# gnlpfjh/Scalable-E3-GNN

Measured on AMD Instinct MI355X. Metric: particles/sec (octree build + SEGNN fwd), 1M pts l_max=2, 1/2/4/8 MI355X, higher is better.
Workload: dtype f32; 1 GPU; 1000000 particles/GPU uniform in unit box, radius graph k~24 (E=23519616), SEGNN l_max=2 4 layers H=32 f32 storage; particles_per_gpu=1000000, edges_per_gpu=23519616, hidden=32, layers=4, lmax=2, parallelism=single GPU

## Files before the change

### include/e3gnn.h

```cpp
#ifndef E3GNN_H
#define E3GNN_H

#include <stdint.h>

#ifdef __cplusplus
extern "C" {
#endif

#define E3GNN_ABI_VERSION 3

enum {
  E3_OK = 0,
  E3_ERR_INVALID_ARG = 1,
  E3_ERR_BAD_IRREPS = 2,
  E3_ERR_MISSING_WEIGHT = 3,
  E3_ERR_UNSUPPORTED = 4,
  E3_ERR_HIP = 5,
  E3_ERR_NO_DEVICE = 6
};

enum { E3_F32 = 0, E3_F64 = 1, E3_BF16 = 2 };

enum { E3_CLS_0E = 0, E3_CLS_0O = 1, E3_CLS_1E = 2, E3_CLS_1O = 3 };

// ... 122 lines not shown
int e3_pow2_scale(const e3_tp_segment* segs, const int64_t* nrows, int nseg, int target_log2, float* out4,
                  void* stream);
int e3_add_pow2_scale(const float* h, const float* u, float* out, int64_t n, int target_log2, float* out4,
                      void* stream);
int e3_tp_forward_fused(const e3_tp_plan* plan, const e3_tp_segment* segs, int nseg,
                        const void* in2, int64_t ld_in2, const void* packed, void* out, int64_t ld_out,
                        int64_t B, int dtype, int gate, const float* in_scale, void* stream);
int e3_tp_forward_fused_epilogue(const e3_tp_plan* plan, const e3_tp_segment* segs, int nseg, const void* in2,
                                 int64_t ld_in2, const void* packed, void* out, int64_t ld_out, int64_t B, int dtype,
                                 int gate, const float* in_scale, const void* residual, int64_t ld_residual,
                                 float* out_scale4, int target_log2, void* stream);
int e3_tp_forward_update_pair(const e3_tp_plan* plan1, const e3_tp_plan* plan2, const e3_tp_segment* segs, int nseg,
                              const void* in2, int64_t ld_in2, const void* packed1, const void* packed2,
                              const float* in_scale, const void* residual, int64_t ld_residual, void* out,
                              int64_t ld_out, int64_t B, int dtype, float* out_scale4, int target_log2, void* stream);
int e3_tp_backward(const e3_tp_plan* plan, const void* in1, int64_t ld_in1, const void* in2, int64_t ld_in2,
                   const void* packed, const void* grad_out, int64_t ld_gout, void* grad_in1, int64_t ld_gin1,
                   void* grad_in2, int64_t ld_gin2, void* const grad_weights[6], int64_t B, int dtype, void* stream);
int e3_tp_backward_weights(const e3_tp_plan* plan, const void* in1, int64_t ld_in1, const void* in2, int64_t ld_in2,
                           const void* packed, const void* grad_out, int64_t ld_gout, void* const grad_weights[6],
                           int64_t B, int dtype, void* stream);
int e3_tp_backward_operands(const e3_tp_plan* plan, const void* in1, int64_t ld_in1, const void* in2, int64_t ld_in2,
                            const void* packed, const void* grad_out, int64_t ld_gout, void* const features[6],
                            void* const gout[6], int64_t B, int dtype, void* stream);
int e3_tp_backward_contract(const e3_tp_plan* plan, const void* in1, int64_t ld_in1, const void* in2, int64_t ld_in2,
                            void* const t[6], void* grad_in1, int64_t ld_gin1, void* grad_in2, int64_t ld_gin2,
                            int64_t B, int dtype, void* stream);
int e3_tp_fused_supported(const e3_tp_plan* plan, int gate);
const char* e3_tp_last_fused_kernel(void);
int e3_tp_forward_fused_scatter(const e3_tp_plan* plan, const e3_tp_segment* segs, int nseg,
// ... 59 lines not shown
```

### scalable-e3-gnn_amd/_lib.py

```python
from __future__ import annotations

import ctypes
import os
from ctypes import POINTER, c_char_p, c_int, c_int32, c_int64, c_void_p

_HERE = os.path.dirname(os.path.abspath(__file__))
LIB_PATH = os.path.join(_HERE, "lib", "libe3gnn_hip.so")

E3_OK = 0
E3_F32, E3_F64, E3_BF16 = 0, 1, 2
CLS_NAMES = ("l0e", "l0o", "l1e", "l1o")

_lib = None

VoidP4 = c_void_p * 4
Float3 = ctypes.c_float * 3
Int3 = c_int32 * 3


class HaloEntry(ctypes.Structure):
    _fields_ = [("lo", ctypes.c_float * 3), ("hi", ctypes.c_float * 3), ("shift", ctypes.c_float * 3)]


SIGNATURES = {
# ... 81 lines not shown
    "e3_pow2_scale": (c_int, [c_void_p, POINTER(c_int64), c_int, c_int, c_void_p, c_void_p]),
    "e3_add_pow2_scale": (c_int, [c_void_p, c_void_p, c_void_p, c_int64, c_int, c_void_p, c_void_p]),
    "e3_tp_backward": (c_int, [c_void_p, c_void_p, c_int64, c_void_p, c_int64, c_void_p, c_void_p, c_int64, c_void_p,
                               c_int64, c_void_p, c_int64, c_void_p * 6, c_int64, c_int, c_void_p]),
    "e3_tp_backward_weights": (c_int, [c_void_p, c_void_p, c_int64, c_void_p, c_int64, c_void_p, c_void_p, c_int64, c_void_p,
                                       c_int64, c_int, c_void_p]),
    "e3_tp_backward_operands": (c_int, [c_void_p, c_void_p, c_int64, c_void_p, c_int64, c_void_p, c_void_p, c_int64, c_void_p,
                                        c_void_p, c_int64, c_int, c_void_p]),
    "e3_tp_backward_contract": (c_int, [c_void_p, c_void_p, c_int64, c_void_p, c_int64, c_void_p, c_void_p, c_int64, c_void_p,
                                        c_int64, c_int64, c_int, c_void_p]),
    "e3_tp_forward_fused_epilogue": (c_int, [c_void_p, c_void_p, c_int, c_void_p, c_int64, c_void_p, c_void_p, c_int64,
                                             c_int64, c_int, c_int, c_void_p, c_void_p, c_int64, c_void_p, c_int, c_void_p]),
    "e3_tp_forward_update_pair": (c_int, [c_void_p, c_void_p, c_void_p, c_int, c_void_p, c_int64, c_void_p, c_void_p,
                                          c_void_p, c_void_p, c_int64, c_void_p, c_int64, c_int64, c_int, c_void_p, c_int,
                                          c_void_p]),
    "e3_tp_fused_supported": (c_int, [c_void_p, c_int]),
    "e3_tp_last_fused_kernel": (ctypes.c_char_p, []),
    "e3_tp_forward_fused_scatter": (c_int, [c_void_p, c_void_p, c_int, c_void_p, c_int64, c_void_p, c_void_p, c_void_p,
                                            c_int64, c_int64, c_int, c_int, c_void_p, c_void_p]),
    "e3_segment_sum_bf16": (c_int, [c_void_p, c_int64, c_void_p, c_int64, c_int, c_void_p, c_int64, c_void_p]),
    "e3_edge_geometry_l2": (c_int, [c_void_p, c_void_p, c_void_p, c_int64, c_void_p, c_void_p, c_void_p, c_void_p]),
    "e3_gate_blocks": (c_int, [c_void_p, c_int64, c_void_p, c_int64, c_int64, c_int, c_int, POINTER(c_int32),
                               POINTER(c_int32), c_void_p]),
    "e3_l1tp_backward": (c_int, [c_void_p, c_void_p, c_int64, c_void_p, c_int64, VoidP4, VoidP4, c_void_p, c_int64,
                                 c_void_p, c_int64, c_void_p, VoidP4, c_void_p, c_int64, c_int, c_void_p]),
    "e3_edge_geometry_strained": (c_int, [c_void_p, c_void_p, c_void_p, c_int64, c_int, POINTER(ctypes.c_float), c_void_p,
                                          c_void_p, c_int, c_void_p, c_void_p, c_void_p, c_void_p]),
    "e3_edge_geometry_backward_strained_workspace_bytes": (c_int64, [c_int64]),
    "e3_edge_geometry_backward_strained": (c_int, [c_void_p, c_void_p, c_void_p, c_int64, c_int, POINTER(ctypes.c_float),
                                                   c_void_p, c_void_p, c_int, c_void_p, c_void_p, c_void_p, c_void_p,
# ... 100 lines not shown
```

### scalable-e3-gnn_amd/csrc/e3_tp.hip

```cpp
#include "e3_common.h"
#include "cg_tables.h"
#include "e3_tp_internal.h"

#include <algorithm>
#include <cstdlib>
#include <map>
#include <mutex>
#include <utility>

namespace e3 {

static int tp_ensure_dyn_lds(const void* fn, size_t bytes) {
  if (bytes <= 64 * 1024) return E3_OK;
  static std::mutex mu;
  static std::map<std::pair<const void*, int>, size_t> have;
  int dev = 0;
  if (hipGetDevice(&dev) != hipSuccess) return E3_ERR_HIP;
  std::lock_guard<std::mutex> lock(mu);
  size_t& cur = have[std::make_pair(fn, dev)];
  if (bytes > cur) {
    if (hipFuncSetAttribute(fn, hipFuncAttributeMaxDynamicSharedMemorySize, (int)bytes) != hipSuccess) return E3_ERR_HIP;
    cur = bytes;
  }
  return E3_OK;
// ... 1112 lines not shown
  if ((dtype != E3_F32 && dtype != E3_BF16) || !plan->fast.usable || ld2 == 0) return E3_ERR_UNSUPPORTED;
  hipStream_t s = (hipStream_t)stream;
  if (out_scale4) E3_HIP_CHECK(hipMemsetAsync(out_scale4, 0, 16, s));
  if (B > 0) {
    if (!in2 || !packed || !out || ld2 < plan->dev.Dy) return E3_ERR_INVALID_ARG;
    int st = tp_ensure_device(plan);
    if (st != E3_OK) return st;
    st = fast_forward(&plan->fast, segs, nseg, plan->dev.D1, in2, ld2, (const char*)packed + fast_section_offset(plan), out,
                      ldo, B, gate, dtype, plan->dev.ocol, in_scale, s, nullptr, residual, ld_residual,
                      out_scale4 ? reinterpret_cast<uint32_t*>(out_scale4) + 2 : nullptr);
    if (st != E3_OK) return st;
  }
  return out_scale4 ? scale_finalize(out_scale4, target_log2, s) : E3_OK;
}

int e3_tp_forward_update_pair(const e3_tp_plan* plan1, const e3_tp_plan* plan2, const e3_tp_segment* segs, int nseg,
                              const void* in2, int64_t ld2, const void* packed1, const void* packed2,
                              const float* in_scale, const void* residual, int64_t ld_residual, void* out, int64_t ldo,
                              int64_t B, int dtype, float* out_scale4, int target_log2, void* stream) {
  if (!plan1 || !plan2 || !segs || B < 0 || (residual && ld_residual <= 0)) return E3_ERR_INVALID_ARG;
  if (out_scale4 && (target_log2 < -20 || target_log2 > 14)) return E3_ERR_INVALID_ARG;
  if ((dtype != E3_F32 && dtype != E3_BF16) || ld2 == 0 || !e3::r16_pair_supported(&plan1->fast, &plan2->fast))
    return E3_ERR_UNSUPPORTED;
  if (!in2 || !packed1 || !packed2 || !out || ld2 < plan1->dev.Dy || ldo < plan2->dev.Dout) return E3_ERR_INVALID_ARG;
  hipStream_t s = (hipStream_t)stream;
  int st = tp_ensure_device(plan1);
  if (st == E3_OK) st = tp_ensure_device(plan2);
  if (st != E3_OK) return st;
  if (out_scale4) E3_HIP_CHECK(hipMemsetAsync(out_scale4, 0, 16, s));
  if (B > 0) {
    st = fast_forward_pair(&plan1->fast, &plan2->fast, segs, nseg, plan1->dev.D1, in2, ld2,
                           (const char*)packed1 + fast_section_offset(plan1), (const char*)packed2 + fast_section_offset(plan2),
                           out, ldo, B, dtype, plan1->dev.ocol, plan2->dev.ocol, in_scale, residual, ld_residual,
                           out_scale4 ? reinterpret_cast<uint32_t*>(out_scale4) + 2 : nullptr, s);
    if (st != E3_OK) return st;
  }
  return out_scale4 ? scale_finalize(out_scale4, target_log2, s) : E3_OK;
}

int e3_tp_forward_fused_scatter(const e3_tp_plan* plan, const e3_tp_segment* segs, int nseg, const void* in2,
                                int64_t ld2, const void* packed, const int32_t* row_node, void* out_nodes,
                                int64_t ldo, int64_t B, int dtype, int gate, const float* in_scale, void* stream) {
  if (!plan || !segs || !row_node || B < 0) return E3_ERR_INVALID_ARG;
  if ((dtype != E3_F32 && dtype != E3_BF16) || !gate || !plan->fast.usable || ld2 == 0) return E3_ERR_UNSUPPORTED;
  if (B == 0) return E3_OK;
  if (!in2 || !packed || !out_nodes || ld2 < plan->dev.Dy) return E3_ERR_INVALID_ARG;
  int st = tp_ensure_device(plan);
  if (st != E3_OK) return st;
  return fast_forward(&plan->fast, segs, nseg, plan->dev.D1, in2, ld2, (const char*)packed + fast_section_offset(plan),
                      out_nodes, ldo, B, gate, dtype, plan->dev.ocol, in_scale, (hipStream_t)stream, row_node);
}

// ... 102 lines not shown
```

### scalable-e3-gnn_amd/csrc/e3_tp_internal.h

```cpp
#pragma once
#include "e3_common.h"

#include <array>
#include <vector>

namespace e3 {

struct TpPath { int c1, l1, l2, wrow; };

struct FChunk {
  int col, count, l1;
  int wblk[3][3];
  int S[2], rows_per[2], inv[2];
};
struct FDev {
  int Dout, Dy, nchunks, ntab, lsh;
  int M[3], NT[3], Mpad[3], ooff[3];
  int bfoff[3];
  int bftotal;
};
struct FPack { int l3, orig_row, count, wblk; };

struct TpFast {
  FDev dev;
// ... 19 lines not shown
                 const float* in_scale, hipStream_t s, const int32_t* scatter = nullptr, const void* residual = nullptr,
                 int64_t ldr = 0, uint32_t* amax = nullptr);
int scale_finalize(float* out4, int target_log2, hipStream_t s);

void fast_note_kernel(const char* name);
const char* fast_last_kernel();

bool fast_gate_shape_ok(const TpFast* F);
bool r16_supported(const TpFast* F);
int fast_forward_r16(const TpFast* F, const void* seg_args, const void* in2, int64_t ld2, const void* packed, void* out,
                     int64_t ldo, int64_t B, int gate, int io16, const int32_t* ocol_tab, const float* in_scale,
                     hipStream_t s);
bool r16_pair_supported(const TpFast* F1, const TpFast* F2);
int fast_forward_pair_r16(const TpFast* F1, const TpFast* F2, const void* seg_args, const void* in2, int64_t ld2,
                          const void* packed1, const void* packed2, void* out, int64_t ldo, int64_t B, int io16,
                          const int32_t* ocol1, const int32_t* ocol2, const float* in_scale, hipStream_t s);
int fast_forward_pair(const TpFast* F1, const TpFast* F2, const e3_tp_segment* segs, int nseg, int D1, const void* in2,
                      int64_t ld2, const void* packed1, const void* packed2, void* out, int64_t ldo, int64_t B, int dtype,
                      const int32_t* ocol1, const int32_t* ocol2, const float* in_scale, const void* residual,
                      int64_t ldr, uint32_t* amax, hipStream_t s);

}
```

### scalable-e3-gnn_amd/csrc/e3_tp_mfma.hip

```cpp
#include "e3_common.h"
#include "e3_tp_internal.h"

#include <algorithm>
#include <cstdlib>
#include <vector>

namespace e3 {

#include "e3_tp_mfma_core.h"

template <typename T>
__global__ void fast_absmax_kernel(const T* w0, int64_t n0, const T* w1, int64_t n1, const T* w2, int64_t n2,
                                   uint32_t* hdr) {
  const T* w[3] = {w0, w1, w2};
  const int64_t n[3] = {n0, n1, n2};
  float m = 0.f;
  for (int c = 0; c < 3; ++c)
    for (int64_t i = blockIdx.x * (int64_t)blockDim.x + threadIdx.x; i < n[c]; i += (int64_t)gridDim.x * blockDim.x)
      m = fmax_finite(m, to_acc(w[c][i]));
  for (int o = 32; o > 0; o >>= 1) m = fmaxf(m, __shfl_xor(m, o));
  if ((threadIdx.x & 63) == 0 && m > 0.f) atomicMax(hdr, __builtin_bit_cast(uint32_t, m));
}

template <typename T>
// ... 197 lines not shown
                 uint32_t* amax) {
  if (!F->usable) return E3_ERR_UNSUPPORTED;
  const bool io16 = dtype == E3_BF16;
  SegArgs sa;
  const int st = fast_seg_args(F, segs, nseg, D1, ldo, scatter, residual, ldr, amax, sa);
  if (st != E3_OK) return st;
  if (gate && !fast_gate_shape_ok(F)) return E3_ERR_UNSUPPORTED;
  const int r = fast_forward_r16(F, &sa, in2, ld2, packed, out, ldo, B, gate, io16 ? 1 : 0, ocol_tab, in_scale, s);
  if (r == 1) return E3_OK;
  return r < 0 ? -r : E3_ERR_UNSUPPORTED;
}

int fast_forward_pair(const TpFast* F1, const TpFast* F2, const e3_tp_segment* segs, int nseg, int D1, const void* in2,
                      int64_t ld2, const void* packed1, const void* packed2, void* out, int64_t ldo, int64_t B, int dtype,
                      const int32_t* ocol1, const int32_t* ocol2, const float* in_scale, const void* residual,
                      int64_t ldr, uint32_t* amax, hipStream_t s) {
  if (!F1->usable || !F2->usable || !r16_pair_supported(F1, F2)) return E3_ERR_UNSUPPORTED;
  SegArgs sa;
  const int st = fast_seg_args(F1, segs, nseg, D1, ldo, nullptr, residual, ldr, amax, sa);
  if (st != E3_OK) return st;
  const int r = fast_forward_pair_r16(F1, F2, &sa, in2, ld2, packed1, packed2, out, ldo, B, dtype == E3_BF16 ? 1 : 0,
                                      ocol1, ocol2, in_scale, s);
  if (r == 1) return E3_OK;
  return r < 0 ? -r : E3_ERR_UNSUPPORTED;
}

}
```

### scalable-e3-gnn_amd/csrc/e3_tp_mfma_r16.hip

```cpp
#include "e3_common.h"
#include "cg_tables.h"
#include "e3_tp_internal.h"

#include <algorithm>
#include <cstdlib>
#include <mutex>
#include <type_traits>
#include <utility>
#include <vector>

namespace e3 {

#include "e3_tp_mfma_core.h"

template <int NT16, bool IO16, int STRIDE>
__device__ __forceinline__ void mma_group(const uint4 (&ah)[NT16], const uint4 (&al)[IO16 ? 1 : NT16], const uint4 bh,
                                          const uint4 bl, f32x4* acc) {
  if constexpr (IO16) {
#pragma unroll
    for (int t = 0; t < NT16; ++t)
      acc[t * STRIDE] = mfma16(__builtin_bit_cast(bf16x8, ah[t]), __builtin_bit_cast(bf16x8, bh), acc[t * STRIDE]);
  } else {
#pragma unroll
    for (int t = 0; t < NT16; ++t)
// ... 35 lines not shown
#pragma unroll
      for (int e = 0; e < 8; ++e) {
        const uint32_t w = w4[e >> 1];
        (&x[0][0])[8 * u + e] = __builtin_bit_cast(float, (e & 1) ? (w & 0xffff0000u) : (w << 16));
      }
    }
  } else {
    const float4* xv = reinterpret_cast<const float4*>(xr + 8 * g * D1);
#pragma unroll
    for (int u = 0; u < 2 * D1; ++u) {
      const float4 v = xv[u];
      (&x[0][0])[4 * u + 0] = v.x * xs; (&x[0][0])[4 * u + 1] = v.y * xs;
      (&x[0][0])[4 * u + 2] = v.z * xs; (&x[0][0])[4 * u + 3] = v.w * xs;
    }
  }
}

template <int L1, int L2, int L3, int NT16, bool IO16>
__device__ __forceinline__ void run16(const float (&x)[8][2 * L1 + 1], const bool live,
                                      const uint4* __restrict__ whi, const uint4* __restrict__ wlo,
                                      const float (&y)[9], f32x4 (&acc)[NT16][2 * L3 + 1]) {
  constexpr int D1 = 2 * L1 + 1, D2 = 2 * L2 + 1, D3 = 2 * L3 + 1;
  using C = CG<L1, L2, L3>;
  __builtin_amdgcn_sched_barrier(0);
  uint4 ah[NT16], al[IO16 ? 1 : NT16];
#pragma unroll
  for (int t = 0; t < NT16; ++t) {
    ah[t] = whi[16 * t];
    if constexpr (!IO16) al[t] = wlo[16 * t];
  }
// ... 431 lines not shown
  }
  if constexpr (!SCAT) {
    if (segs.amax) {
#pragma unroll
      for (int o = 32; o > 0; o >>= 1) amax = fmaxf(amax, __shfl_xor(amax, o, 64));
      if (lane == 0 && amax > 0.f) atomicMax(segs.amax, __builtin_bit_cast(uint32_t, amax));
    }
  }
}

struct PairArgs {
  const float* packed;
  const FDev* dp;
  const FChunk* chunks;
  const int32_t* ocol_tab;
};
constexpr int kPairTarget = 10;

template <int LSH, int NT0, int NT1, int NT2, int MODE, int... L1S>
__global__ __launch_bounds__(256, 2) void tp_update_pair_r16_kernel(SegArgs segs, const float* __restrict__ in2, int64_t ld2,
                                                                    const float* __restrict__ packed,
                                                                    void* __restrict__ outv, int64_t ldo, int64_t B,
                                                                    const FDev* __restrict__ dp,
                                                                    const FChunk* __restrict__ chunks,
                                                                    const int32_t* __restrict__ ocol_tab,
                                                                    const float* __restrict__ in_scale, PairArgs pr) {
  constexpr bool IO16 = MODE == 2;
  constexpr int NL = (NT1 > 0 ? 1 : 0) + (NT2 > 0 ? 1 : 0);
  static_assert(NT1 == 1 && NT2 <= 1 && NT0 == 1 + NL, "hidden 32: scalars and one gate block per degree, one tile each");
  constexpr int CHUNK = r16_chunk(r16_max({L1S...}), NL);
// ... 94 lines not shown
    stage(0);

    f32x4 a0[2 * NT0][1], a1[2][3], a2[NT2 > 0 ? 2 : 1][5];
#pragma unroll
    for (int t = 0; t < 2 * NT0; ++t) a0[t][0] = f32x4{0, 0, 0, 0};
#pragma unroll
    for (int t = 0; t < 2; ++t)
#pragma unroll
      for (int c = 0; c < 3; ++c) a1[t][c] = f32x4{0, 0, 0, 0};
#pragma unroll
    for (int t = 0; t < (NT2 > 0 ? 2 : 1); ++t)
#pragma unroll
      for (int c = 0; c < 5; ++c) a2[t][c] = f32x4{0, 0, 0, 0};
    float y[9];
    int ci = 0;
    auto process = [&](auto itag) {
      constexpr int L1 = Seq::at(decltype(itag)::value);
      wait_vm0();
      wave_sync_lds();
      if (ci == 0) {
#pragma unroll
        for (int q = 0; q < 9; ++q) y[q] = (q < Dy) ? ybuf[j * Dy + q] : 0.f;
      }
      const FChunk ch = chunks[ci];
      float x[8][2 * L1 + 1];
      load_x16<L1, IO16>(cbuf + j * (((32 * (2 * L1 + 1) / (IO16 ? 8 : 4)) | 1) * 4), g, xs, x);
#define E3_RUN(L2v, L3v, ACC, NTv)                                                                             \
  if constexpr (Slots::valid(L1, L2v, L3v)) {                                                                  \
    const size_t o = (size_t)(cBfoff[L3v] >> 3) + (size_t)(2 * ch.wblk[L2v][L3v] + g) * cMpad[L3v] + j;        \
    run16<L1, L2v, L3v, 2 * NTv, IO16>(x, true, whi_base + o, wlo_base + o, y, ACC);                            \
  }
      E3_RUN(0, 0, a0, NT0) E3_RUN(1, 0, a0, NT0) E3_RUN(2, 0, a0, NT0)
      E3_RUN(0, 1, a1, NT1) E3_RUN(1, 1, a1, NT1) E3_RUN(2, 1, a1, NT1)
      E3_RUN(0, 2, a2, NT2) E3_RUN(1, 2, a2, NT2) E3_RUN(2, 2, a2, NT2)
#undef E3_RUN
      wave_sync_lds();
      if (ci + 1 < nchunks) stage(ci + 1);
      ++ci;
    };
    for_each_index(process, std::make_index_sequence<sizeof...(L1S)>{});
    wait_vm0();
    wave_sync_lds();

    {
      const float* nrm0 = nrm + ocl[cOoff[0]];
#pragma unroll
      for (int q = 0; q < 8; ++q) {
        const float s = a0[q >> 2][0][q & 3] * nrm0[chan_of(q)];
        a0[q >> 2][0][q & 3] = s * sigmoid_(s);
      }
      const float* nv1 = nrm + ocl[cOoff[1]];
#pragma unroll
      for (int q = 0; q < 8; ++q) {
        const float gq = sigmoid_(a0[2 + (q >> 2)][0][q & 3] * nrm0[32 + chan_of(q)]);
#pragma unroll
        for (int c = 0; c < 3; ++c) a1[q >> 2][c][q & 3] = (gq * a1[q >> 2][c][q & 3]) * nv1[3 * chan_of(q) + c];
      }
      if constexpr (NT2 > 0) {
        const float* nv2 = nrm + ocl[cOoff[2]];
#pragma unroll
        for (int q = 0; q < 8; ++q) {
          const float gq = sigmoid_(a0[4 + (q >> 2)][0][q & 3] * nrm0[64 + chan_of(q)]);
#pragma unroll
          for (int c = 0; c < 5; ++c) a2[q >> 2][c][q & 3] = (gq * a2[q >> 2][c][q & 3]) * nv2[5 * chan_of(q) + c];
        }
      }
    }
    float srow = 1.0f, isrow = 1.0f;
    if constexpr (!IO16) {
      float m = 0.f;
#pragma unroll
      for (int q = 0; q < 8; ++q) {
        m = fmax_finite(m, a0[q >> 2][0][q & 3]);
#pragma unroll
        for (int c = 0; c < 3; ++c) m = fmax_finite(m, a1[q >> 2][c][q & 3]);
        if constexpr (NT2 > 0) {
#pragma unroll
          for (int c = 0; c < 5; ++c) m = fmax_finite(m, a2[q >> 2][c][q & 3]);
        }
      }
      m = fmaxf(m, __shfl_xor(m, 16, 64));
      m = fmaxf(m, __shfl_xor(m, 32, 64));
      srow = pow2_scale_from_bits(__builtin_bit_cast(uint32_t, m), kPairTarget);
      isrow = 1.0f / srow;
    }

    f32x4 b0[2][1], b1[2][3], b2[NT2 > 0 ? 2 : 1][5];
#pragma unroll
    for (int t = 0; t < 2; ++t) {
      b0[t][0] = f32x4{0, 0, 0, 0};
#pragma unroll
      for (int c = 0; c < 3; ++c) b1[t][c] = f32x4{0, 0, 0, 0};
    }
#pragma unroll
    for (int t = 0; t < (NT2 > 0 ? 2 : 1); ++t)
#pragma unroll
      for (int c = 0; c < 5; ++c) b2[t][c] = f32x4{0, 0, 0, 0};
    auto put = [&](auto dtag, auto val) {
      constexpr int D = decltype(dtag)::value;
// ... 261 lines not shown
  const FDev& d = F1->dev;
  const FDev& d2 = F2->dev;
  const size_t tables =
      (size_t)(((d.Dout + 15) & ~15) + ((d.ntab + 15) & ~15) + ((d2.Dout + 15) & ~15) + ((d2.ntab + 15) & ~15)) * 4;
  int lin = 0;
  for (auto& c : F1->h_chunks) lin = std::max(lin, c.l1);
  return tables + nwaves * (size_t)(r16_chunk(lin, d.NT[2] > 0 ? 2 : 1) + 160) * 4;
}

bool r16_pair_supported(const TpFast* F1, const TpFast* F2) {
  return r16_find(F1) != nullptr && r16_pair_find(F1, F2) != nullptr && 2 * r16_pair_lds_bytes(F1, F2, kR16Waves) <= (size_t)kFastLds;
}

int fast_forward_pair_r16(const TpFast* F1, const TpFast* F2, const void* sa_, const void* in2, int64_t ld2,
                          const void* packed1, const void* packed2, void* out, int64_t ldo, int64_t B, int io16,
                          const int32_t* ocol1, const int32_t* ocol2, const float* in_scale, hipStream_t s) {
  const SegArgs& sa = *static_cast<const SegArgs*>(sa_);
  const R16PairEntry* e = r16_pair_find(F1, F2);
  if (!e || sa.scatter) return 0;
  const int epu = io16 ? 8 : 4;
  for (int i = 0; i < sa.nseg; ++i)
    if (sa.index[i] || (sa.ld[i] % epu) || ((sa.col0[i + 1] - sa.col0[i]) % epu) ||
        (reinterpret_cast<uintptr_t>(sa.base[i]) & 15))
      return 0;
  const void* fn = e->fn[io16 ? 1 : 0];
  const size_t lds_bytes = r16_pair_lds_bytes(F1, F2, kR16Waves);
  if (2 * lds_bytes > (size_t)kFastLds) return 0;
  {
    int dev = 0;
    if (hipGetDevice(&dev) != hipSuccess) return -E3_ERR_HIP;
    static std::mutex mu;
    static std::vector<std::pair<const void*, int>> configured;
    std::lock_guard<std::mutex> lock(mu);
    if (std::find(configured.begin(), configured.end(), std::make_pair(fn, dev)) == configured.end()) {
      if (hipFuncSetAttribute(fn, hipFuncAttributeMaxDynamicSharedMemorySize, (int)lds_bytes) != hipSuccess) return -E3_ERR_HIP;
      configured.emplace_back(fn, dev);
    }
  }
  const int64_t ntiles = (B + 15) / 16;
  const int grid = (int)std::min<int64_t>((ntiles + kR16Waves - 1) / kR16Waves, 256 * 2);
  const float* in2f = (const float*)in2;
  const float* pk = (const float*)packed1;
  void* outf = out;
  const FDev* dd = F1->d_dev;
  const FChunk* dc = F1->d_chunks;
  PairArgs pa{(const float*)packed2, F2->d_dev, F2->d_chunks, ocol2};
  void* args[] = {const_cast<void*>(sa_), &in2f, &ld2, &pk, &outf, &ldo, &B, &dd, &dc, &ocol1, &in_scale, &pa};
  if (hipLaunchKernel(fn, dim3(grid), dim3(64 * kR16Waves), args, lds_bytes, s) != hipSuccess) return -E3_ERR_HIP;
  fast_note_kernel("e3::tp_update_pair_r16_kernel");
  return 1;
}

}
```

### scalable-e3-gnn_amd/segnn.py

```python
from __future__ import annotations

import torch
from torch import nn

from . import ops
from .irreps import Irreps
from .l1_tensor_prod import L1TensorProduct
from .message import FusedMessage
from .radius_graph import RadiusGraph
from .tensor_product import SHTensorProduct


def _hidden_irreps(H: int, lmax: int):
    hid = Irreps(f"{H}x0e+{H}x1o" + (f"+{H}x2e" if lmax == 2 else ""))
    gated = Irreps(f"{H}x0e+{lmax * H}x0e+{H}x1o" + (f"+{H}x2e" if lmax == 2 else ""))
    return hid, gated


def _make_tp(in_irreps, out_irreps, lmax: int):
    if lmax == 1:
        if Irreps(in_irreps).lmax == 1 and Irreps(out_irreps).lmax == 1:
            return L1TensorProduct(in_irreps, out_irreps)
        return SHTensorProduct(in_irreps, out_irreps, lmax_sh=1)
    return SHTensorProduct(in_irreps, out_irreps, lmax_sh=2)
# ... 75 lines not shown
            m = self.msg1.forward_fused([(h, g.dst), (h, g.src), (d, None)], Y, gate=True,
                                        in_scale=ops.pow2_scale([h, d]) if f32 else None)
            a = None
            if self.fuse_scatter:
                a = self.msg2.forward_fused([(m, None)], Y, gate=True, scatter=(g.dst, g.rowptr.numel() - 1))
            if a is None:
                m = self.msg2.forward_fused([(m, None)], Y, gate=True)
                a = ops.segment_sum(m, g)
        else:
            m = ops.gather_concat(h, g, d)
            m = self._gate(self.msg1(m, Y))
            m = self._gate(self.msg2(m, Y))
            a = ops.segment_sum(m, g)
        if r16u:
            sc = None
            if f32 and h_scale is not None and halo is None:
                sc = ops.join_pow2_scales(h_scale, ops.pow2_scale([a]))
            if self.upd2.fused_supported(False) and h.stride(-1) == 1:
                if isinstance(self.upd1, SHTensorProduct) and a.stride(-1) == 1:
                    r = self.upd1.forward_update_pair(self.upd2, [(h, None), (a, None)], A, in_scale=sc, residual=h,
                                                      out_scale=10 if f32 else None)
                    if r is not None:
                        return r if f32 else (r, None)
                u, u_scale = self.upd1.forward_fused([(h, None), (a, None)], A, gate=True, in_scale=sc,
                                                     out_scale=10 if f32 else None) if f32 else \
                    (self.upd1.forward_fused([(h, None), (a, None)], A, gate=True), None)
                if f32:
                    return self.upd2.forward_fused([(u, None)], A, gate=False, in_scale=u_scale, residual=h, out_scale=10)
                return self.upd2.forward_fused([(u, None)], A, gate=False, residual=h), None
            u = self.upd1.forward_fused([(h, None), (a, None)], A, gate=True, in_scale=sc)
        else:
            u = self._gate(self.upd1(torch.cat([h, a], 1), A))
        u = self.upd2(u, A)
        if f32 and inference:
            return ops.add_pow2_scale(h, u)
        return h + u, None


# ... 45 lines not shown
```

### scalable-e3-gnn_amd/tensor_product.py

```python
from __future__ import annotations

import ctypes
from math import sqrt

import torch
from torch import nn

from . import _lib, profiling
from .irreps import Irreps, as_blocks

CLASSES = ("l0e", "l0o", "l1e", "l1o", "l2e", "l2o")


class TPSegment(ctypes.Structure):
    _fields_ = [("base", ctypes.c_void_p), ("ld", ctypes.c_int64), ("row_index", ctypes.c_void_p),
                ("ncols", ctypes.c_int32), ("reserved", ctypes.c_int32)]


class TPPlan:

    def __init__(self, in1_irreps, out_irreps, lmax_sh):
        lib = _lib.load()
        self._blocks = ([tuple(b) for b in as_blocks(in1_irreps)], int(lmax_sh), [tuple(b) for b in as_blocks(out_irreps)])
        self._plans = _lib.DevicePlans("e3_tp_plan_create", "e3_tp_plan_destroy", *self._blocks)
# ... 158 lines not shown
            else:
                _lib.check(lib.e3_tp_forward_fused(h, ctypes.byref(segs), len(segments), in2.data_ptr(),
                                                   in2.stride(0), packed.data_ptr(), out.data_ptr(), out.stride(0), B,
                                                   _lib.dtype_code(io), 1 if gate else 0, sc, stream), "e3_tp_forward_fused")
            if t0 is not None:
                nb = sum((t.shape[0] * t.shape[1] * esz + (4 * B if idx is not None else 0)) for t, idx in
                         [(k, s[1]) for k, s in zip(keep, segments)]) + 4 * self.in2_dim * B + \
                     (esz * width * B if scatter is None else 4 * B + 4 * width * scatter[1])
                mode = "<bf16 storage, bf16 MFMA>" if io == torch.bfloat16 else "<fp16x3 split MFMA>"
                profiling.end(f"tp_fused{'+segsum' if scatter is not None else ''} {tag} B={B}", B, nb, t0, flops=self.flops_per_row * B,
                              kernel=(lib.e3_tp_last_fused_kernel() or b"e3::tp_fwd_mfma_r16_kernel").decode() + mode)
        if out_scale is not None:
            return out, sc4
        return out

    def forward_update_pair(self, ws, ns, plan2, ws2, ns2, segments, in2, in_scale=None, residual=None, out_scale=None):
        lib = _lib.load()
        B = in2.shape[0]
        dev = in2.device
        io = segments[0][0].dtype
        if io not in (torch.float32, torch.bfloat16) or in2.dtype != torch.float32 or in2.stride(-1) != 1:
            return None
        segs = (TPSegment * len(segments))()
        keep = []
        for i, (t, idx) in enumerate(segments):
            if idx is not None or t.dtype != io or t.stride(-1) != 1 or t.shape[0] != B:
                return None
            keep.append(t)
            segs[i].base, segs[i].ld, segs[i].ncols = t.data_ptr(), t.stride(0), t.shape[1]
        out = torch.empty((B, plan2.out_dim), dtype=io, device=dev)
        if residual is not None and (residual.shape != out.shape or residual.dtype != io or residual.stride(-1) != 1):
            raise RuntimeError(f"forward_update_pair: residual must be {tuple(out.shape)} {io}, contiguous rows")
        with torch.cuda.device(dev):
            h1, h2 = self.handle(dev), plan2.handle(dev)
            packed1 = self.packed(ws, ns, io, dev)
            packed2 = plan2.packed(ws2, ns2, io, dev)
            if io == torch.float32 and in_scale is None:
                from . import ops
                in_scale = ops.pow2_scale(keep)
            sc = in_scale.data_ptr() if (in_scale is not None and io == torch.float32) else None
            sc4 = torch.empty(4, dtype=torch.float32, device=dev) if out_scale is not None else None
            stream = torch.cuda.current_stream(dev).cuda_stream
            t0 = profiling.begin() if profiling.enabled() else None
            st = lib.e3_tp_forward_update_pair(
                h1, h2, ctypes.byref(segs), len(segments), in2.data_ptr(), in2.stride(0), packed1.data_ptr(),
                packed2.data_ptr(), sc, residual.data_ptr() if residual is not None else None,
                residual.stride(0) if residual is not None else 0, out.data_ptr(), out.stride(0), B, _lib.dtype_code(io),
                sc4.data_ptr() if sc4 is not None else None, int(out_scale) if out_scale is not None else 0, stream)
            if st == 4:
                return None
            _lib.check(st, "e3_tp_forward_update_pair")
            if t0 is not None:
                esz = out.element_size()
                nb = sum(t.numel() * esz for t in keep) + 4 * self.in2_dim * B + esz * out.numel() * (2 if residual is not None else 1)
                mode = "<bf16 storage, bf16 MFMA>" if io == torch.bfloat16 else "<fp16x3 split MFMA>"
                profiling.end(f"tp_update_pair B={B}", B, nb, t0, flops=(self.flops_per_row + plan2.flops_per_row) * B,
                              kernel=(lib.e3_tp_last_fused_kernel() or b"e3::tp_update_pair_r16_kernel").decode() + mode)
        if out_scale is not None:
            return out, sc4
        return out


def _rebuild_tpplan(in_blocks, lmax_sh, out_blocks):
# ... 145 lines not shown
        ns = [getattr(self, "norm_" + c) for c in CLASSES]
        return ws, ns

    def _packed_weights(self, dtype, device):
        ws, ns = self._tensors()
        return self._plan.packed(ws, ns, dtype, device)

    def fused_supported(self, gate: bool) -> bool:
        return self._plan.fused_supported(gate)

    def forward_fused(self, segments, in2, gate: bool = False, scatter=None, in_scale=None, residual=None, out_scale=None):
        ws, ns = self._tensors()
        return self._plan.forward_fused(ws, ns, segments, in2, gate, tag=f"{self.iri1}->{self.iro}", scatter=scatter,
                                        in_scale=in_scale, residual=residual, out_scale=out_scale)

    def forward_update_pair(self, second, segments, in2, in_scale=None, residual=None, out_scale=None):
        ws, ns = self._tensors()
        ws2, ns2 = second._tensors()
        return self._plan.forward_update_pair(ws, ns, second._plan, ws2, ns2, segments, in2, in_scale=in_scale,
                                              residual=residual, out_scale=out_scale)

    def forward(self, in1: torch.Tensor, in2: torch.Tensor) -> torch.Tensor:
        torch._assert(in1.shape[-1] == self.in1_dim,
                      f"Incorrect last dimension for in1 = {in1.shape[-1]}, required is {self.in1_dim}")
        torch._assert(in2.shape[-1] == self.in2_dim,
                      f"Incorrect last dimension for in2 = {in2.shape[-1]}, required is {self.in2_dim}")
        if not in1.is_cuda:
            raise RuntimeError("SHTensorProduct runs on ROCm tensors only; there is no CPU path")
        if torch.is_grad_enabled() and (in1.requires_grad or in2.requires_grad or
                                        any(p.requires_grad for p in self.parameters())):
            if in1.dtype not in (torch.float32, torch.float64):
                raise NotImplementedError("SHTensorProduct backward: float32 / float64 only")
            if in1.stride(-1) != 1:
                in1 = in1.contiguous()
            if in2.stride(-1) != 1:
# ... 39 lines not shown
```

Before: 11.31 million particles/s.

## Compute per-row pow2 input scaling inside fused update-pair kernel

Adds a row-scale mode to the fused update-pair TP kernel. The kernel derives the power-of-two input scale on the fly from a running absmax of each loaded chunk and rescales the accumulators when the scale changes. This lets the f32 SEGNN update path skip the separate pow2_scale/join_pow2_scales kernels that previously computed a global input scale before the fused call. It also swaps the absmax loops for v_max3 asm and replaces the reciprocal division with a bit-trick pow2 inverse, at the cost of extra in-kernel ballot and rescale work.

```diff
diff --git a/include/e3gnn.h b/include/e3gnn.h
--- a/include/e3gnn.h
+++ b/include/e3gnn.h
@@ -160,6 +160,11 @@
                               const void* in2, int64_t ld_in2, const void* packed1, const void* packed2,
                               const float* in_scale, const void* residual, int64_t ld_residual, void* out,
                               int64_t ld_out, int64_t B, int dtype, float* out_scale4, int target_log2, void* stream);
+int e3_tp_forward_update_pair_rowscale(const e3_tp_plan* plan1, const e3_tp_plan* plan2, const e3_tp_segment* segs,
+                                       int nseg, const void* in2, int64_t ld_in2, const void* packed1,
+                                       const void* packed2, const void* residual, int64_t ld_residual, void* out,
+                                       int64_t ld_out, int64_t B, int dtype, float* out_scale4, int target_log2,
+                                       void* stream);
 int e3_tp_backward(const e3_tp_plan* plan, const void* in1, int64_t ld_in1, const void* in2, int64_t ld_in2,
                    const void* packed, const void* grad_out, int64_t ld_gout, void* grad_in1, int64_t ld_gin1,
                    void* grad_in2, int64_t ld_gin2, void* const grad_weights[6], int64_t B, int dtype, void* stream);
diff --git a/scalable-e3-gnn_amd/_lib.py b/scalable-e3-gnn_amd/_lib.py
--- a/scalable-e3-gnn_amd/_lib.py
+++ b/scalable-e3-gnn_amd/_lib.py
@@ -119,6 +119,9 @@
     "e3_tp_forward_update_pair": (c_int, [c_void_p, c_void_p, c_void_p, c_int, c_void_p, c_int64, c_void_p, c_void_p,
                                           c_void_p, c_void_p, c_int64, c_void_p, c_int64, c_int64, c_int, c_void_p, c_int,
                                           c_void_p]),
+    "e3_tp_forward_update_pair_rowscale": (c_int, [c_void_p, c_void_p, c_void_p, c_int, c_void_p, c_int64, c_void_p,
+                                                   c_void_p, c_void_p, c_int64, c_void_p, c_int64, c_int64, c_int,
+                                                   c_void_p, c_int, c_void_p]),
     "e3_tp_fused_supported": (c_int, [c_void_p, c_int]),
     "e3_tp_last_fused_kernel": (ctypes.c_char_p, []),
     "e3_tp_forward_fused_scatter": (c_int, [c_void_p, c_void_p, c_int, c_void_p, c_int64, c_void_p, c_void_p, c_void_p,
diff --git a/scalable-e3-gnn_amd/csrc/e3_tp.hip b/scalable-e3-gnn_amd/csrc/e3_tp.hip
--- a/scalable-e3-gnn_amd/csrc/e3_tp.hip
+++ b/scalable-e3-gnn_amd/csrc/e3_tp.hip
@@ -1150,10 +1150,10 @@
   return out_scale4 ? scale_finalize(out_scale4, target_log2, s) : E3_OK;
 }
 
-int e3_tp_forward_update_pair(const e3_tp_plan* plan1, const e3_tp_plan* plan2, const e3_tp_segment* segs, int nseg,
-                              const void* in2, int64_t ld2, const void* packed1, const void* packed2,
-                              const float* in_scale, const void* residual, int64_t ld_residual, void* out, int64_t ldo,
-                              int64_t B, int dtype, float* out_scale4, int target_log2, void* stream) {
+static int tp_update_pair(const e3_tp_plan* plan1, const e3_tp_plan* plan2, const e3_tp_segment* segs, int nseg,
+                          const void* in2, int64_t ld2, const void* packed1, const void* packed2, const float* in_scale,
+                          int row_scale, const void* residual, int64_t ld_residual, void* out, int64_t ldo, int64_t B,
+                          int dtype, float* out_scale4, int target_log2, void* stream) {
   if (!plan1 || !plan2 || !segs || B < 0 || (residual && ld_residual <= 0)) return E3_ERR_INVALID_ARG;
   if (out_scale4 && (target_log2 < -20 || target_log2 > 14)) return E3_ERR_INVALID_ARG;
   if ((dtype != E3_F32 && dtype != E3_BF16) || ld2 == 0 || !e3::r16_pair_supported(&plan1->fast, &plan2->fast))
@@ -1168,10 +1168,26 @@
     st = fast_forward_pair(&plan1->fast, &plan2->fast, segs, nseg, plan1->dev.D1, in2, ld2,
                            (const char*)packed1 + fast_section_offset(plan1), (const char*)packed2 + fast_section_offset(plan2),
                            out, ldo, B, dtype, plan1->dev.ocol, plan2->dev.ocol, in_scale, residual, ld_residual,
-                           out_scale4 ? reinterpret_cast<uint32_t*>(out_scale4) + 2 : nullptr, s);
+                           out_scale4 ? reinterpret_cast<uint32_t*>(out_scale4) + 2 : nullptr, row_scale, s);
     if (st != E3_OK) return st;
   }
   return out_scale4 ? scale_finalize(out_scale4, target_log2, s) : E3_OK;
+}
+
+int e3_tp_forward_update_pair(const e3_tp_plan* plan1, const e3_tp_plan* plan2, const e3_tp_segment* segs, int nseg,
+                              const void* in2, int64_t ld2, const void* packed1, const void* packed2,
+                              const float* in_scale, const void* residual, int64_t ld_residual, void* out, int64_t ldo,
+                              int64_t B, int dtype, float* out_scale4, int target_log2, void* stream) {
+  return tp_update_pair(plan1, plan2, segs, nseg, in2, ld2, packed1, packed2, in_scale, 0, residual, ld_residual, out, ldo,
+                        B, dtype, out_scale4, target_log2, stream);
+}
+
+int e3_tp_forward_update_pair_rowscale(const e3_tp_plan* plan1, const e3_tp_plan* plan2, const e3_tp_segment* segs,
+                                       int nseg, const void* in2, int64_t ld2, const void* packed1, const void* packed2,
+                                       const void* residual, int64_t ld_residual, void* out, int64_t ldo, int64_t B,
+                                       int dtype, float* out_scale4, int target_log2, void* stream) {
+  return tp_update_pair(plan1, plan2, segs, nseg, in2, ld2, packed1, packed2, nullptr, 1, residual, ld_residual, out, ldo,
+                        B, dtype, out_scale4, target_log2, stream);
 }
 
 int e3_tp_forward_fused_scatter(const e3_tp_plan* plan, const e3_tp_segment* segs, int nseg, const void* in2,
diff --git a/scalable-e3-gnn_amd/csrc/e3_tp_internal.h b/scalable-e3-gnn_amd/csrc/e3_tp_internal.h
--- a/scalable-e3-gnn_amd/csrc/e3_tp_internal.h
+++ b/scalable-e3-gnn_amd/csrc/e3_tp_internal.h
@@ -57,10 +57,10 @@
 bool r16_pair_supported(const TpFast* F1, const TpFast* F2);
 int fast_forward_pair_r16(const TpFast* F1, const TpFast* F2, const void* seg_args, const void* in2, int64_t ld2,
                           const void* packed1, const void* packed2, void* out, int64_t ldo, int64_t B, int io16,
-                          const int32_t* ocol1, const int32_t* ocol2, const float* in_scale, hipStream_t s);
+                          const int32_t* ocol1, const int32_t* ocol2, const float* in_scale, int row_scale, hipStream_t s);
 int fast_forward_pair(const TpFast* F1, const TpFast* F2, const e3_tp_segment* segs, int nseg, int D1, const void* in2,
                       int64_t ld2, const void* packed1, const void* packed2, void* out, int64_t ldo, int64_t B, int dtype,
                       const int32_t* ocol1, const int32_t* ocol2, const float* in_scale, const void* residual,
-                      int64_t ldr, uint32_t* amax, hipStream_t s);
+                      int64_t ldr, uint32_t* amax, int row_scale, hipStream_t s);
 
 }
diff --git a/scalable-e3-gnn_amd/csrc/e3_tp_mfma.hip b/scalable-e3-gnn_amd/csrc/e3_tp_mfma.hip
--- a/scalable-e3-gnn_amd/csrc/e3_tp_mfma.hip
+++ b/scalable-e3-gnn_amd/csrc/e3_tp_mfma.hip
@@ -235,13 +235,13 @@
 int fast_forward_pair(const TpFast* F1, const TpFast* F2, const e3_tp_segment* segs, int nseg, int D1, const void* in2,
                       int64_t ld2, const void* packed1, const void* packed2, void* out, int64_t ldo, int64_t B, int dtype,
                       const int32_t* ocol1, const int32_t* ocol2, const float* in_scale, const void* residual,
-                      int64_t ldr, uint32_t* amax, hipStream_t s) {
+                      int64_t ldr, uint32_t* amax, int row_scale, hipStream_t s) {
   if (!F1->usable || !F2->usable || !r16_pair_supported(F1, F2)) return E3_ERR_UNSUPPORTED;
   SegArgs sa;
   const int st = fast_seg_args(F1, segs, nseg, D1, ldo, nullptr, residual, ldr, amax, sa);
   if (st != E3_OK) return st;
   const int r = fast_forward_pair_r16(F1, F2, &sa, in2, ld2, packed1, packed2, out, ldo, B, dtype == E3_BF16 ? 1 : 0,
-                                      ocol1, ocol2, in_scale, s);
+                                      ocol1, ocol2, in_scale, row_scale, s);
   if (r == 1) return E3_OK;
   return r < 0 ? -r : E3_ERR_UNSUPPORTED;
 }
diff --git a/scalable-e3-gnn_amd/csrc/e3_tp_mfma_r16.hip b/scalable-e3-gnn_amd/csrc/e3_tp_mfma_r16.hip
--- a/scalable-e3-gnn_amd/csrc/e3_tp_mfma_r16.hip
+++ b/scalable-e3-gnn_amd/csrc/e3_tp_mfma_r16.hip
@@ -73,6 +73,29 @@
       (&x[0][0])[4 * u + 2] = v.z * xs; (&x[0][0])[4 * u + 3] = v.w * xs;
     }
   }
+}
+
+__device__ __forceinline__ float max3_abs(float m, float a, float b) {
+  float r;
+  asm("v_max3_f32 %0, %1, |%2|, |%3|" : "=v"(r) : "v"(m), "v"(a), "v"(b));
+  return r;
+}
+template <int N>
+__device__ __forceinline__ float absmax_finite(const float* v, const float m) {
+  static_assert(N % 2 == 0, "pairs");
+  float r = m;
+#pragma unroll
+  for (int e = 0; e < N; e += 2) r = max3_abs(r, v[e], v[e + 1]);
+  if (!(r < INFINITY)) {
+    r = m;
+#pragma unroll
+    for (int e = 0; e < N; ++e) r = fmax_finite(r, v[e]);
+  }
+  return r;
+}
+__device__ __forceinline__ float pow2_inverse(const float s) {
+  const uint32_t b = 0x7f000000u - __builtin_bit_cast(uint32_t, s);
+  return __builtin_bit_cast(float, b > 0x00400000u ? b : 0x00400000u);
 }
 
 template <int L1, int L2, int L3, int NT16, bool IO16>
@@ -534,6 +557,7 @@
   const FDev* dp;
   const FChunk* chunks;
   const int32_t* ocol_tab;
+  int row_scale;
 };
 constexpr int kPairTarget = 10;
 
@@ -658,6 +682,7 @@
       for (int c = 0; c < 5; ++c) a2[t][c] = f32x4{0, 0, 0, 0};
     float y[9];
     int ci = 0;
+    float m1 = 0.f, s1 = 1.0f, is1 = 1.0f;
     auto process = [&](auto itag) {
       constexpr int L1 = Seq::at(decltype(itag)::value);
       wait_vm0();
@@ -668,7 +693,39 @@
       }
       const FChunk ch = chunks[ci];
       float x[8][2 * L1 + 1];
-      load_x16<L1, IO16>(cbuf + j * (((32 * (2 * L1 + 1) / (IO16 ? 8 : 4)) | 1) * 4), g, xs, x);
+      load_x16<L1, IO16>(cbuf + j * (((32 * (2 * L1 + 1) / (IO16 ? 8 : 4)) | 1) * 4), g, 1.0f, x);
+      if constexpr (!IO16) {
+        float sx = xs;
+        if (pr.row_scale) {
+          float m = absmax_finite<8 * (2 * L1 + 1)>(&x[0][0], m1);
+          m = fmaxf(m, __shfl_xor(m, 16, 64));
+          m = fmaxf(m, __shfl_xor(m, 32, 64));
+          m1 = m;
+          const float sn = pow2_scale_from_bits(__builtin_bit_cast(uint32_t, m), kPairTarget);
+          if (ci > 0 && __builtin_amdgcn_ballot_w64(sn != s1) != 0) {
+            const float ratio = sn * is1;
+#pragma unroll
+            for (int t = 0; t < 2 * NT0; ++t) a0[t][0] *= ratio;
+#pragma unroll
+            for (int t = 0; t < 2; ++t)
+#pragma unroll
+              for (int c = 0; c < 3; ++c) a1[t][c] *= ratio;
+            if constexpr (NT2 > 0) {
+#pragma unroll
+              for (int t = 0; t < 2; ++t)
+#pragma unroll
+                for (int c = 0; c < 5; ++c) a2[t][c] *= ratio;
+            }
+          }
+          s1 = sn;
+          is1 = pow2_inverse(sn);
+          sx = sn;
+        }
+#pragma unroll
+        for (int i = 0; i < 8; ++i)
+#pragma unroll
+          for (int u = 0; u < 2 * L1 + 1; ++u) x[i][u] *= sx;
+      }
 #define E3_RUN(L2v, L3v, ACC, NTv)                                                                             \
   if constexpr (Slots::valid(L1, L2v, L3v)) {                                                                  \
     const size_t o = (size_t)(cBfoff[L3v] >> 3) + (size_t)(2 * ch.wblk[L2v][L3v] + g) * cMpad[L3v] + j;        \
@@ -688,45 +745,41 @@
 
     {
       const float* nrm0 = nrm + ocl[cOoff[0]];
+      auto un1 = [&](float v) {
+        if constexpr (IO16) return v;
+        else return v * is1;
+      };
 #pragma unroll
       for (int q = 0; q < 8; ++q) {
-        const float s = a0[q >> 2][0][q & 3] * nrm0[chan_of(q)];
+        const float s = un1(a0[q >> 2][0][q & 3]) * nrm0[chan_of(q)];
         a0[q >> 2][0][q & 3] = s * sigmoid_(s);
       }
       const float* nv1 = nrm + ocl[cOoff[1]];
 #pragma unroll
       for (int q = 0; q < 8; ++q) {
-        const float gq = sigmoid_(a0[2 + (q >> 2)][0][q & 3] * nrm0[32 + chan_of(q)]);
-#pragma unroll
-        for (int c = 0; c < 3; ++c) a1[q >> 2][c][q & 3] = (gq * a1[q >> 2][c][q & 3]) * nv1[3 * chan_of(q) + c];
+        const float gq = sigmoid_(un1(a0[2 + (q >> 2)][0][q & 3]) * nrm0[32 + chan_of(q)]);
+#pragma unroll
+        for (int c = 0; c < 3; ++c) a1[q >> 2][c][q & 3] = (gq * un1(a1[q >> 2][c][q & 3])) * nv1[3 * chan_of(q) + c];
       }
       if constexpr (NT2 > 0) {
         const float* nv2 = nrm + ocl[cOoff[2]];
 #pragma unroll
         for (int q = 0; q < 8; ++q) {
-          const float gq = sigmoid_(a0[4 + (q >> 2)][0][q & 3] * nrm0[64 + chan_of(q)]);
-#pragma unroll
-          for (int c = 0; c < 5; ++c) a2[q >> 2][c][q & 3] = (gq * a2[q >> 2][c][q & 3]) * nv2[5 * chan_of(q) + c];
+          const float gq = sigmoid_(un1(a0[4 + (q >> 2)][0][q & 3]) * nrm0[64 + chan_of(q)]);
+#pragma unroll
+          for (int c = 0; c < 5; ++c) a2[q >> 2][c][q & 3] = (gq * un1(a2[q >> 2][c][q & 3])) * nv2[5 * chan_of(q) + c];
         }
       }
     }
     float srow = 1.0f, isrow = 1.0f;
     if constexpr (!IO16) {
-      float m = 0.f;
-#pragma unroll
-      for (int q = 0; q < 8; ++q) {
-        m = fmax_finite(m, a0[q >> 2][0][q & 3]);
-#pragma unroll
-        for (int c = 0; c < 3; ++c) m = fmax_finite(m, a1[q >> 2][c][q & 3]);
-        if constexpr (NT2 > 0) {
-#pragma unroll
-          for (int c = 0; c < 5; ++c) m = fmax_finite(m, a2[q >> 2][c][q & 3]);
-        }
-      }
+      float m = absmax_finite<8>(reinterpret_cast<const float*>(&a0[0][0]), 0.f);
+      m = absmax_finite<24>(reinterpret_cast<const float*>(&a1[0][0]), m);
+      if constexpr (NT2 > 0) m = absmax_finite<40>(reinterpret_cast<const float*>(&a2[0][0]), m);
       m = fmaxf(m, __shfl_xor(m, 16, 64));
       m = fmaxf(m, __shfl_xor(m, 32, 64));
       srow = pow2_scale_from_bits(__builtin_bit_cast(uint32_t, m), kPairTarget);
-      isrow = 1.0f / srow;
+      isrow = pow2_inverse(srow);
     }
 
     f32x4 b0[2][1], b1[2][3], b2[NT2 > 0 ? 2 : 1][5];
@@ -1018,7 +1071,7 @@
 
 int fast_forward_pair_r16(const TpFast* F1, const TpFast* F2, const void* sa_, const void* in2, int64_t ld2,
                           const void* packed1, const void* packed2, void* out, int64_t ldo, int64_t B, int io16,
-                          const int32_t* ocol1, const int32_t* ocol2, const float* in_scale, hipStream_t s) {
+                          const int32_t* ocol1, const int32_t* ocol2, const float* in_scale, int row_scale, hipStream_t s) {
   const SegArgs& sa = *static_cast<const SegArgs*>(sa_);
   const R16PairEntry* e = r16_pair_find(F1, F2);
   if (!e || sa.scatter) return 0;
@@ -1048,7 +1101,8 @@
   void* outf = out;
   const FDev* dd = F1->d_dev;
   const FChunk* dc = F1->d_chunks;
-  PairArgs pa{(const float*)packed2, F2->d_dev, F2->d_chunks, ocol2};
+  PairArgs pa{(const float*)packed2, F2->d_dev, F2->d_chunks, ocol2, (row_scale && !io16) ? 1 : 0};
+  if (pa.row_scale) in_scale = nullptr;
   void* args[] = {const_cast<void*>(sa_), &in2f, &ld2, &pk, &outf, &ldo, &B, &dd, &dc, &ocol1, &in_scale, &pa};
   if (hipLaunchKernel(fn, dim3(grid), dim3(64 * kR16Waves), args, lds_bytes, s) != hipSuccess) return -E3_ERR_HIP;
   fast_note_kernel("e3::tp_update_pair_r16_kernel");
diff --git a/scalable-e3-gnn_amd/segnn.py b/scalable-e3-gnn_amd/segnn.py
--- a/scalable-e3-gnn_amd/segnn.py
+++ b/scalable-e3-gnn_amd/segnn.py
@@ -113,14 +113,15 @@
             a = ops.segment_sum(m, g)
         if r16u:
             sc = None
+            if self.upd2.fused_supported(False) and h.stride(-1) == 1:
+                if isinstance(self.upd1, SHTensorProduct) and a.stride(-1) == 1:
+                    r = self.upd1.forward_update_pair(self.upd2, [(h, None), (a, None)], A, residual=h,
+                                                      out_scale=10 if f32 else None, row_scale=f32)
+                    if r is not None:
+                        return r if f32 else (r, None)
             if f32 and h_scale is not None and halo is None:
                 sc = ops.join_pow2_scales(h_scale, ops.pow2_scale([a]))
             if self.upd2.fused_supported(False) and h.stride(-1) == 1:
-                if isinstance(self.upd1, SHTensorProduct) and a.stride(-1) == 1:
-                    r = self.upd1.forward_update_pair(self.upd2, [(h, None), (a, None)], A, in_scale=sc, residual=h,
-                                                      out_scale=10 if f32 else None)
-                    if r is not None:
-                        return r if f32 else (r, None)
                 u, u_scale = self.upd1.forward_fused([(h, None), (a, None)], A, gate=True, in_scale=sc,
                                                      out_scale=10 if f32 else None) if f32 else \
                     (self.upd1.forward_fused([(h, None), (a, None)], A, gate=True), None)
diff --git a/scalable-e3-gnn_amd/tensor_product.py b/scalable-e3-gnn_amd/tensor_product.py
--- a/scalable-e3-gnn_amd/tensor_product.py
+++ b/scalable-e3-gnn_amd/tensor_product.py
@@ -196,7 +196,8 @@
             return out, sc4
         return out
 
-    def forward_update_pair(self, ws, ns, plan2, ws2, ns2, segments, in2, in_scale=None, residual=None, out_scale=None):
+    def forward_update_pair(self, ws, ns, plan2, ws2, ns2, segments, in2, in_scale=None, residual=None, out_scale=None,
+                            row_scale=False):
         lib = _lib.load()
         B = in2.shape[0]
         dev = in2.device
@@ -217,18 +218,23 @@
             h1, h2 = self.handle(dev), plan2.handle(dev)
             packed1 = self.packed(ws, ns, io, dev)
             packed2 = plan2.packed(ws2, ns2, io, dev)
-            if io == torch.float32 and in_scale is None:
+            row_scale = bool(row_scale) and io == torch.float32
+            if io == torch.float32 and in_scale is None and not row_scale:
                 from . import ops
                 in_scale = ops.pow2_scale(keep)
             sc = in_scale.data_ptr() if (in_scale is not None and io == torch.float32) else None
             sc4 = torch.empty(4, dtype=torch.float32, device=dev) if out_scale is not None else None
             stream = torch.cuda.current_stream(dev).cuda_stream
             t0 = profiling.begin() if profiling.enabled() else None
-            st = lib.e3_tp_forward_update_pair(
-                h1, h2, ctypes.byref(segs), len(segments), in2.data_ptr(), in2.stride(0), packed1.data_ptr(),
-                packed2.data_ptr(), sc, residual.data_ptr() if residual is not None else None,
-                residual.stride(0) if residual is not None else 0, out.data_ptr(), out.stride(0), B, _lib.dtype_code(io),
-                sc4.data_ptr() if sc4 is not None else None, int(out_scale) if out_scale is not None else 0, stream)
+            tail = (residual.data_ptr() if residual is not None else None,
+                    residual.stride(0) if residual is not None else 0, out.data_ptr(), out.stride(0), B, _lib.dtype_code(io),
+                    sc4.data_ptr() if sc4 is not None else None, int(out_scale) if out_scale is not None else 0, stream)
+            head = (h1, h2, ctypes.byref(segs), len(segments), in2.data_ptr(), in2.stride(0), packed1.data_ptr(),
+                    packed2.data_ptr())
+            if row_scale:
+                st = lib.e3_tp_forward_update_pair_rowscale(*head, *tail)
+            else:
+                st = lib.e3_tp_forward_update_pair(*head, sc, *tail)
             if st == 4:
                 return None
             _lib.check(st, "e3_tp_forward_update_pair")
@@ -404,11 +410,11 @@
         return self._plan.forward_fused(ws, ns, segments, in2, gate, tag=f"{self.iri1}->{self.iro}", scatter=scatter,
                                         in_scale=in_scale, residual=residual, out_scale=out_scale)
 
-    def forward_update_pair(self, second, segments, in2, in_scale=None, residual=None, out_scale=None):
+    def forward_update_pair(self, second, segments, in2, in_scale=None, residual=None, out_scale=None, row_scale=False):
         ws, ns = self._tensors()
         ws2, ns2 = second._tensors()
         return self._plan.forward_update_pair(ws, ns, second._plan, ws2, ns2, segments, in2, in_scale=in_scale,
-                                              residual=residual, out_scale=out_scale)
+                                              residual=residual, out_scale=out_scale, row_scale=row_scale)
 
     def forward(self, in1: torch.Tensor, in2: torch.Tensor) -> torch.Tensor:
         torch._assert(in1.shape[-1] == self.in1_dim,
```

Result: no change. 11.41 million particles/s (median of 6 runs) (+0.9%).
